# safijari/yag-slam

Measured on AMD Instinct MI355X. Metric: pose hypotheses/sec, higher is better.
Workload: dtype u8

## Files before the change

include/yagmatch.h:

```cpp
#ifndef YAGMATCH_H
#define YAGMATCH_H

#include <stdint.h>

#ifdef __cplusplus
extern "C" {
#endif

#define YM_VERSION 1

enum {
    YM_OK = 0,
    YM_ERR_INVALID = -1,
    YM_ERR_NO_DEVICE = -2,
    YM_ERR_HIP = -3,
    YM_ERR_UNSUPPORTED = -4,
    YM_ERR_RANGE = -5,
    YM_ERR_BUSY = -6
};

enum { YM_SEM_KARTO = 0, YM_SEM_YAGPY = 1 };

typedef struct ym_config {
    double angle_variance_penalty;
// ... 269 lines not shown
void ym_graph_destroy(ym_graph *g);
int ym_graph_add_nodes(ym_graph *g, const double *xyt, int n);
int ym_graph_add_constraints(ym_graph *g, const int32_t *from_to, const double *mean_xyt, const double *info9, int n);
int ym_graph_size(const ym_graph *g, int32_t *nodes, int32_t *constraints);
int ym_graph_set_poses(ym_graph *g, int first, const double *xyt, int n);
int ym_graph_get_poses(const ym_graph *g, int first, double *xyt, int n);
int ym_graph_hold(ym_graph *g, const int32_t *nodes, int n, int hold );
int ym_graph_held(const ym_graph *g, uint8_t *mask, int n_nodes);
int ym_graph_chi2(ym_graph *g, double *chi2);
int ym_graph_linearise(ym_graph *g, double *chi2, double *diag9 , double *grad3 );
int ym_graph_solve(ym_graph *g, int band , double lambda, double cg_tol, int max_cg_iters ,
                   double *delta3 , double *precond3 , int32_t *band_used,
                   int32_t *cg_iterations, double *residual, int32_t *flags);
typedef struct ym_opt_params { int32_t iters, exact, max_cg_iters, band ; double lambda0, cg_tol; } ym_opt_params;
typedef struct ym_opt_report { double chi2_initial, chi2_final, lambda_final; int32_t lm_steps, accepted, cg_iterations, band, status; } ym_opt_report;
int ym_graph_optimize(ym_graph *g, const ym_opt_params *p, ym_opt_report *out);

enum { YM_ROBUST_NONE = 0, YM_ROBUST_HUBER = 1, YM_ROBUST_CAUCHY = 2, YM_ROBUST_GEMAN_MCCLURE = 3 };
int ym_graph_set_robust(ym_graph *g, const int32_t *edges, int n, int kind, double param);
int ym_graph_enable(ym_graph *g, const int32_t *edges, int n, int enable );
int ym_graph_edge_terms(ym_graph *g, double *s , double *w );
int ym_graph_cost(ym_graph *g, double *cost);

typedef struct ym_grid_info {
    int32_t width, height, pitch;
    int32_t origin_x, origin_y;
    int32_t storage_w, storage_h;
    int32_t roi_x, roi_y, roi_w, roi_h;
    double offset_x, offset_y;
} ym_grid_info;
int ym_debug_grid_info(ym_matcher *m, int item, ym_grid_info *info);
int ym_debug_grid(ym_matcher *m, int item, uint8_t *out, int64_t out_bytes);
int ym_debug_sums(ym_matcher *m, int item, int pass, uint32_t *out, int64_t out_count);
int ym_debug_map_sums(ym_matcher *m, int item, int pass, uint32_t *out, int64_t out_count);
int ym_debug_query_local(ym_matcher *m, int item, double *out_xy, int32_t cap, int32_t *n);
int ym_debug_cells(ym_matcher *m, int item, int32_t *out, int64_t out_count, int32_t *max_n);
typedef struct ym_pair_list_info {
    int32_t nt, lnw, lparts, nbins;
    int32_t nrx, nry, nregions;
    int32_t rg_h, rg_cls, rg_zero;
    int32_t ng;
    int32_t qrep, cx0, cy0, nq;
    int32_t n_slots;
    int64_t entries_pstride;
    double off_x, off_y;
    double ylat[2];
} ym_pair_list_info;
int ym_debug_pair_lists(ym_matcher *m, int slot, ym_pair_list_info *info, double *ctrig, int32_t *starts, int32_t *flags,
                        uint16_t *entries, uint32_t *rbox);

int ym_debug_option(ym_matcher *m, int option, int value);

#define YM_DEBUG_COUNTERS 10
int ym_debug_counters(ym_matcher *m, int64_t *out, int32_t count);

int ym_debug_live_bytes(int64_t *device_bytes, int64_t *pinned_bytes);

int ym_debug_stamps(ym_matcher *m, int enable, uint64_t *out, int32_t count);

int ym_profile_enable(ym_matcher *m, int on);
int ym_profile_read(ym_matcher *m, int which, double *ms_total, int64_t *launches, int reset);
int ym_cache_stats(const ym_matcher *m, int64_t *hits, int64_t *misses);

#ifdef __cplusplus
}
#endif
// ... 2 lines not shown
```

yag_slam_amd/_capi.py:

```python
import ctypes as C
import os
import subprocess

_HERE = os.path.dirname(os.path.abspath(__file__))
LIB_PATH = os.environ.get("YM_LIB_PATH") or os.path.join(_HERE, "libyagmatch.so")

YM_OK = 0
SEM = {"karto": 0, "yagpy": 1}

EXPORTS = (
    "ym_version", "ym_build_id", "ym_device_count", "ym_last_error", "ym_create", "ym_destroy", "ym_get_config",
    "ym_set_stream", "ym_synchronize", "ym_scan_create", "ym_scans_create", "ym_scans_destroy", "ym_scan_set_pose", "ym_scans_set_poses", "ym_scan_get_pose",
    "ym_scan_size", "ym_scan_structure_trusted", "ym_scan_destroy", "ym_match", "ym_match_scans", "ym_map_sequence", "ym_process_scan", "ym_sequence_stats", "ym_async_slots",
    "ym_match_scans_async", "ym_wait", "ym_match_batch", "ym_batch_create", "ym_batch_destroy", "ym_batch_size",
    "ym_match_pairs", "ym_pairs_create",
    "ym_batch_run_async", "ym_batch_wait", "ym_debug_grid_info",
    "ym_debug_grid", "ym_debug_sums", "ym_debug_query_local", "ym_debug_cells", "ym_debug_pair_lists", "ym_debug_option", "ym_debug_stamps", "ym_debug_live_bytes",
    "ym_profile_enable",
    "ym_profile_read", "ym_cache_stats", "ym_debug_counters",
    "ym_coarse_dims", "ym_match_slice_begin", "ym_match_slice_finish",
    "ym_occupancy_create", "ym_occupancy_create_counted", "ym_occupancy_get_info", "ym_occupancy_read", "ym_occupancy_read_counts",
    "ym_occupancy_destroy", "ym_image_despeckle", "ym_occupancy_create_clean", "ym_occupancy_get_despeckle_stats",
    "ym_occmap_create", "ym_occmap_accumulate", "ym_occmap_clear", "ym_occmap_get_info", "ym_occmap_read", "ym_occmap_read_counts",
    "ym_occmap_debug_option", "ym_occmap_destroy",
    "ym_map_from_occupancy", "ym_map_from_grid", "ym_map_size", "ym_map_read", "ym_map_destroy", "ym_match_map",
    "ym_match_map_many", "ym_map_track", "ym_debug_map_sums", "ym_match_sets", "ym_match_sets_many",
    "ym_map_create_empty", "ym_map_add_scans", "ym_map_clear",
    "ym_map_create_counted", "ym_map_update_scans", "ym_map_counted", "ym_map_read_stamps",
    "ym_map_reframe", "ym_map_window", "ym_map_create_counted_window",
    "ym_raymap_create", "ym_raymap_trace", "ym_raymap_trace_each", "ym_raymap_destroy",
    "ym_locator_create", "ym_locator_get_info", "ym_locator_read_level", "ym_locator_locate", "ym_locator_destroy",
    "ym_segments_create", "ym_segments_label_range", "ym_segments_stats", "ym_segments_boundaries", "ym_segments_pairs",
    "ym_segments_destroy", "ym_map_free_space", "ym_segments_from_map", "ym_segments_labels",
    "ym_graph_create", "ym_graph_destroy", "ym_graph_add_nodes", "ym_graph_add_constraints", "ym_graph_size", "ym_graph_set_poses",
    "ym_graph_get_poses", "ym_graph_chi2", "ym_graph_linearise", "ym_graph_solve", "ym_graph_optimize",
    "ym_graph_hold", "ym_graph_held", "ym_graph_set_robust", "ym_graph_enable", "ym_graph_edge_terms", "ym_graph_cost",
)


class YmError(RuntimeError):
    def __init__(self, code, msg):
        super().__init__("libyagmatch error %d: %s" % (code, msg))
        self.code = code


class YmConfig(C.Structure):
    _fields_ = [
        ("angle_variance_penalty", C.c_double),
        ("distance_variance_penalty", C.c_double),
        ("coarse_search_angle_offset", C.c_double),
# ... 176 lines not shown
    L.ym_synchronize.argtypes = [vp]
    L.ym_scan_create.restype = vp
    L.ym_scan_create.argtypes = [C.c_int, C.POINTER(YmScanDesc)]
    L.ym_scan_set_pose.argtypes = [vp, C.c_double, C.c_double, C.c_double]
    L.ym_scans_set_poses.argtypes = [C.POINTER(vp), dp, C.c_int]
    L.ym_scan_get_pose.argtypes = [vp, dp]
    L.ym_scan_size.argtypes = [vp]
    L.ym_scan_destroy.argtypes = [vp]
    L.ym_scans_create.argtypes = [C.c_int, vp, C.c_int, vp]
    L.ym_scans_destroy.argtypes = [vp, C.c_int]
    L.ym_scans_destroy.restype = None
    L.ym_scan_destroy.restype = None
    L.ym_match.argtypes = [vp, C.POINTER(YmScanDesc), C.POINTER(YmScanDesc), C.c_int, C.c_int, C.c_int,
                           C.POINTER(YmResult)]
    L.ym_match_scans.argtypes = [vp, vp, C.POINTER(vp), C.c_int, C.c_int, C.c_int, C.POINTER(YmResult)]
    L.ym_async_slots.argtypes = [vp]
    L.ym_match_scans_async.argtypes = [vp, vp, C.POINTER(vp), C.c_int, C.c_int, C.c_int, C.c_int]
    L.ym_wait.argtypes = [vp, C.c_int, C.POINTER(YmResult)]
    L.ym_match_batch.argtypes = [vp, vp, C.POINTER(vp), ip, C.c_int, C.c_int, C.c_int, C.POINTER(YmResult),
                                 C.POINTER(YmResult), ip]
    L.ym_batch_create.restype = vp
    L.ym_batch_create.argtypes = [vp, vp, C.POINTER(vp), ip, C.c_int]
    L.ym_pairs_create.restype = vp
    L.ym_pairs_create.argtypes = [vp, C.POINTER(vp), C.POINTER(vp), ip, C.c_int]
    L.ym_match_pairs.argtypes = [vp, C.POINTER(vp), C.POINTER(vp), ip, C.c_int, C.c_int, C.c_int, C.POINTER(YmResult)]
    L.ym_batch_destroy.argtypes = [vp]
    L.ym_batch_destroy.restype = None
    L.ym_batch_size.argtypes = [vp]
    L.ym_batch_run_async.argtypes = [vp, vp, C.c_int, C.c_int, C.c_int, C.c_int64, vp]
    L.ym_batch_wait.argtypes = [vp, C.c_int, C.POINTER(YmResult), C.POINTER(YmResult), ip]
    L.ym_debug_grid_info.argtypes = [vp, C.c_int, C.POINTER(YmGridInfo)]
    L.ym_debug_grid.argtypes = [vp, C.c_int, C.POINTER(C.c_uint8), C.c_int64]
    L.ym_debug_sums.argtypes = [vp, C.c_int, C.c_int, C.POINTER(C.c_uint32), C.c_int64]
    L.ym_debug_query_local.argtypes = [vp, C.c_int, dp, C.c_int32, ip]
    L.ym_debug_cells.argtypes = [vp, C.c_int, ip, C.c_int64, ip]
    L.ym_debug_pair_lists.argtypes = [vp, C.c_int, C.POINTER(YmPairListInfo), dp, ip, ip, C.POINTER(C.c_uint16), C.POINTER(C.c_uint32)]
    L.ym_debug_option.argtypes = [vp, C.c_int, C.c_int]
    L.ym_debug_stamps.argtypes = [vp, C.c_int, C.POINTER(C.c_uint64), C.c_int32]
    L.ym_debug_live_bytes.argtypes = [C.POINTER(C.c_int64), C.POINTER(C.c_int64)]
    L.ym_profile_enable.argtypes = [vp, C.c_int]
    L.ym_profile_read.argtypes = [vp, C.c_int, dp, C.POINTER(C.c_int64), C.c_int]
    L.ym_cache_stats.argtypes = [vp, C.POINTER(C.c_int64), C.POINTER(C.c_int64)]
    L.ym_debug_counters.argtypes = [vp, C.POINTER(C.c_int64), C.c_int32]
    L.ym_coarse_dims.argtypes = [vp, ip]
    L.ym_scan_structure_trusted.argtypes = [vp, C.c_int]
    L.ym_process_scan.argtypes = [vp, vp, C.POINTER(vp), C.c_int, dp, dp, C.c_int, C.c_int, C.POINTER(YmResult)]
    L.ym_sequence_stats.argtypes = [vp, C.POINTER(C.c_int64), C.POINTER(C.c_int64), C.POINTER(C.c_int64)]
    L.ym_map_sequence.argtypes = [vp, C.POINTER(vp), dp, C.c_int, C.c_int, C.c_int, C.c_int, C.c_int, C.c_int, C.POINTER(YmResult), ip]
    L.ym_match_slice_begin.argtypes = [vp, vp, C.POINTER(vp), C.c_int, C.c_int, C.c_int, C.c_int, C.c_int, vp, vp]
    L.ym_match_slice_finish.argtypes = [vp, C.POINTER(YmResult)]
    L.ym_occupancy_create.restype = vp
    L.ym_occupancy_create.argtypes = [C.POINTER(vp), C.c_int, C.c_double, C.c_double]
    L.ym_occupancy_create_counted.restype = vp
    L.ym_occupancy_create_counted.argtypes = [C.POINTER(vp), C.c_int, C.c_double, C.c_double]
    L.ym_occupancy_get_info.argtypes = [vp, C.POINTER(YmOccupancyInfo)]
    L.ym_occupancy_read.argtypes = [vp, C.POINTER(C.c_uint8), C.c_int64]
    L.ym_occupancy_read_counts.argtypes = [vp, C.POINTER(C.c_uint32), C.POINTER(C.c_uint32), C.c_int64]
    L.ym_occupancy_destroy.argtypes = [vp]
    L.ym_occupancy_destroy.restype = None
    L.ym_image_despeckle.argtypes = [C.c_int, C.POINTER(C.c_uint8), C.c_int, C.c_int, C.c_int, C.POINTER(YmDespeckleOpts),
                                     C.POINTER(C.c_uint8), C.POINTER(YmDespeckleStats)]
    L.ym_occupancy_create_clean.restype = vp
    L.ym_occupancy_create_clean.argtypes = [C.POINTER(vp), C.c_int, C.c_double, C.c_double, C.POINTER(YmDespeckleOpts)]
    L.ym_occupancy_get_despeckle_stats.argtypes = [vp, C.POINTER(YmDespeckleStats)]
    L.ym_occmap_create.restype = vp
    L.ym_occmap_create.argtypes = [C.c_int, C.c_double, C.c_double, dp, C.c_int]
# ... 117 lines not shown
```

yag_slam_amd/csrc/ym_abi_debug.hpp:

```cpp
int ym_debug_map_sums(ym_matcher *m, int item, int pass, uint32_t *out, int64_t out_count);
static bool sets_debug(const ym_matcher *m) { return !m->last_valid && m->map_last.valid && m->sets_last.valid; }
int ym_debug_grid_info(ym_matcher *m, int item, ym_grid_info *info) {
    if (!m || !info) return set_err(YM_ERR_INVALID, "null argument");
    if (sets_debug(m)) {
        const ym_matcher::SetsLast &sl = m->sets_last;
        if (item < 0 || item >= m->map_last.n_items) return set_err(YM_ERR_INVALID, "no such item in the last call");
        std::memset(info, 0, sizeof *info);
        info->width = info->height = info->pitch = sl.G;
        info->storage_w = info->storage_h = info->roi_w = info->roi_h = sl.G;
        YmItemState s;
        DEV_GUARD(m->device);
        HIP_TRY(hipStreamSynchronize(m->stream));
        HIP_TRY(hipMemcpy(&s, m->states.p + item, sizeof s, hipMemcpyDeviceToHost));
        info->offset_x = s.off_x; info->offset_y = s.off_y;
        return YM_OK;
    }
    if (!m->last_valid || item < 0 || item >= m->last_B) return set_err(YM_ERR_INVALID, "no such item in the last call");
    const YmGeom &g = m->last_geom;
    info->width = g.win_w; info->height = g.win_w; info->pitch = g.pitch;
    info->origin_x = g.win_origin; info->origin_y = g.win_origin;
    info->storage_w = g.storage_w; info->storage_h = g.storage_w;
    info->roi_x = g.border; info->roi_y = g.border; info->roi_w = g.roi_w; info->roi_h = g.roi_w;
    YmItemState s;
    DEV_GUARD(m->device);
// ... 8 lines not shown
    if (sets_debug(m)) {
        const ym_matcher::SetsLast &sl = m->sets_last;
        if (item < 0 || item >= m->map_last.n_items) return set_err(YM_ERR_INVALID, "no such item in the last call");
        if (item < sl.first_grid) return set_err(YM_ERR_INVALID, "the grid of item %d was overwritten: the call keeps those of its last chunk, from item %d on", item, sl.first_grid);
        const int64_t need_s = (int64_t)sl.G * sl.G;
        if (out_bytes < need_s) return set_err(YM_ERR_INVALID, "grid buffer too small: need %lld bytes", (long long)need_s);
        DEV_GUARD(m->device);
        HIP_TRY(hipStreamSynchronize(m->stream));
        HIP_TRY(hipMemcpy(out, m->sets_grid.p + (size_t)(item - sl.first_grid) * sl.grid_stride, (size_t)need_s, hipMemcpyDeviceToHost));
        return YM_OK;
    }
    if (!m->last_valid || item < 0 || item >= m->last_B) return set_err(YM_ERR_INVALID, "no such item in the last call");
    const int64_t need = (int64_t)m->last_geom.pitch * m->last_geom.win_w;
    if (out_bytes < need) return set_err(YM_ERR_INVALID, "grid buffer too small: need %lld bytes", (long long)need);
    DEV_GUARD(m->device);
    HIP_TRY(hipStreamSynchronize(m->stream));
    HIP_TRY(hipMemcpy(out, m->grid.p + (size_t)item * m->last_grid_stride, (size_t)need, hipMemcpyDeviceToHost));
    return YM_OK;
}

int ym_debug_sums(ym_matcher *m, int item, int pass, uint32_t *out, int64_t out_count) {
    if (!m || !out || pass < 0 || pass > 1) return set_err(YM_ERR_INVALID, "bad argument");
    if (sets_debug(m)) return ym_debug_map_sums(m, item, pass, out, out_count);
    if (!m->last_valid || item < 0 || item >= m->last_B) return set_err(YM_ERR_INVALID, "no such item in the last call");
    const size_t n = m->last_sums_stride[pass];
    if (n == 0) return set_err(YM_ERR_INVALID, "pass %d did not run", pass);
    const size_t ncopy = std::min(n, (size_t)out_count);
    if (m->cfg.semantics == YM_SEM_KARTO && (size_t)out_count < n)
        return set_err(YM_ERR_INVALID, "sums buffer too small: need %zu entries", n);
    DEV_GUARD(m->device);
    HIP_TRY(hipStreamSynchronize(m->stream));
    HIP_TRY(hipMemcpy(out, m->sums.p + m->sums_pass_offset[pass] + (size_t)item * n, ncopy * sizeof(uint32_t),
                      hipMemcpyDeviceToHost));
    return YM_OK;
}

int ym_debug_query_local(ym_matcher *m, int item, double *out_xy, int32_t cap, int32_t *n) {
    if (!m || !out_xy || !n) return set_err(YM_ERR_INVALID, "null argument");
    const bool sets = sets_debug(m);
    if (sets ? (item < 0 || item >= m->map_last.n_items) : (!m->last_valid || item < 0 || item >= m->last_B))
        return set_err(YM_ERR_INVALID, "no such item in the last call");
    YmItemState s;
    DEV_GUARD(m->device);
    HIP_TRY(hipStreamSynchronize(m->stream));
    HIP_TRY(hipMemcpy(&s, m->states.p + item, sizeof s, hipMemcpyDeviceToHost));
    *n = s.nq;
    if (cap < s.nq) return set_err(YM_ERR_INVALID, "buffer too small: need %d points", s.nq);
    if (s.nq > 0)
        HIP_TRY(hipMemcpy(out_xy, s.ql, sizeof(double2) * s.nq, hipMemcpyDeviceToHost));
    return YM_OK;
}

int ym_debug_cells(ym_matcher *m, int item, int32_t *out, int64_t out_count, int32_t *max_n) {
    if (!m || !max_n) return set_err(YM_ERR_INVALID, "null argument");
    if (!m->last_valid || item < 0 || item >= m->last_B) return set_err(YM_ERR_INVALID, "no such item in the last call");
    *max_n = m->last_max_n;
    const size_t per = (size_t)m->last_max_base * m->last_max_n;
    if (!out) return YM_OK;
    if ((size_t)out_count < per * 2) return set_err(YM_ERR_INVALID, "buffer too small: need %zu ints", per * 2);
    DEV_GUARD(m->device);
    HIP_TRY(hipStreamSynchronize(m->stream));
    std::vector<YmCell> dev(per);
    HIP_TRY(hipMemcpy(dev.data(), m->cells.p + (size_t)item * per, sizeof(YmCell) * per, hipMemcpyDeviceToHost));
    for (size_t i = 0; i < per; i++) {
        const int2 c = ym_cell_unpack(dev[i]);
        out[2 * i] = c.x;
// ... 201 lines not shown
```

yag_slam_amd/csrc/ym_host_call.hpp:

```cpp
int launch_call_body(ym_matcher *m, Slot &slot) {
    static const bool debug_host = getenv("YM_DEBUG_HOST") != nullptr;
    timespec t_[8];
    auto mark = [&](int i) { if (debug_host) clock_gettime(CLOCK_MONOTONIC, &t_[i]); };
    mark(7);
    DEV_GUARD(m->device);
    CallPlan P;
    int rc;
    mark(0);
    m->last_corr_form = -1;
    m->lists_last.valid = false;
    if ((rc = plan_sizes(m, slot, P))) return rc;
    mark(1);
    Call &pc = slot.call;
    const bool replay = pc.batch_uid != 0 && pc.plan_clean && pc.plan_gen == m->cache_gen && pc.pose_epoch == g_pose_epoch.load(std::memory_order_relaxed);
    if (!replay && (rc = plan_cache(m, slot, P))) return rc;
    mark(2);
    if ((rc = plan_jobs(m, slot, P, replay))) return rc;
    mark(3);
    if ((rc = plan_descriptor(m, slot, P, replay))) return rc;
    if (pc.batch_uid != 0 && !replay) {
        bool clean = !m->cache_off;
        for (const CallScan &cs : pc.scans) clean = clean && !cs.stale && !cs.qstale;
        pc.plan_clean = clean;
        pc.plan_gen = m->cache_gen;
// ... 42 lines not shown
        emark(4);
        if (!slot.call.slice) enqueue_finish(m, slot, P);
        else slot.plan = P;
        emark(5);
    }
    if (slot.dev_best_out)
        hipLaunchKernelGGL(ym::argbest_kernel, dim3(1), dim3(256), 0, st, m->states.p, P.B, (long long)slot.chain_id_base,
                           reinterpret_cast<double *>(slot.dev_best_out));
    HIP_TRY(hipGetLastError());
    if ((rc = prof_end(m, ev_call))) return rc;
    if (!slot.done) HIP_TRY(hipEventCreateWithFlags(&slot.done, hipEventDisableTiming));
    if (!slot.call.chain_step) HIP_TRY(hipEventRecord(slot.done, st));
    slot.in_flight = true;
    slot.n_items = P.B;
    HIP_TRY(hipGetLastError());
    mark(6);
    if (debug_host) {
        auto us = [&](int a, int b) { return (t_[b].tv_sec - t_[a].tv_sec) * 1e6 + (t_[b].tv_nsec - t_[a].tv_nsec) * 1e-3; };
        fprintf(stderr, "[ym] host us: guard %.1f sizes %.0f cache %.0f jobs %.0f descriptor %.0f raster-plan %.0f enqueue %.0f (B %d, %d scans)\n", us(7, 0), us(0, 1), us(1, 2),
                us(2, 3), us(3, 4), us(4, 5), us(5, 6), P.B, P.nscans);
        auto eus = [&](int a, int b) { return (e_[b].tv_sec - e_[a].tv_sec) * 1e6 + (e_[b].tv_nsec - e_[a].tv_nsec) * 1e-3; };
        fprintf(stderr, "[ym] enqueue us: prepare %.1f raster %.1f correlate %.1f score %.1f finish %.1f\n", eus(0, 1), eus(1, 2), eus(2, 3), eus(3, 4), eus(4, 5));
    }

    m->last_geom = P.g;
    m->last_lat[0] = P.lc;
    m->last_lat[1] = P.lf;
    m->last_B = P.B; m->last_max_n = P.max_n; m->last_max_base = P.max_base;
    m->last_nt_stride = P.nt_stride; m->last_dim_stride = P.dim_stride;
    m->last_grid_stride = P.grid_stride;
    m->last_sums_stride[0] = P.yag ? P.yvol : (m->keep_sums || (P.B < 8 && P.sums_c <= 65536)) ? P.sums_c : 0;
    m->last_sums_stride[1] = slot.call.refine ? (P.yag ? P.yvol : P.sums_f) : 0;
    m->last_valid = true;
    if (P.region26 && P.k_end > P.k_begin) {
        const ym::RegionArgs r = region_args(m, P);
        ym_matcher::ListsLast &ll = m->lists_last;
        ll.nt = P.lc.nt; ll.lnw = r.nw; ll.lparts = r.parts; ll.nbins = r.nbins; ll.nrx = r.nrx; ll.nry = r.nry; ll.nregions = r.nregions;
        ll.rg_h = r.rg_h; ll.rg_cls = r.rg_cls; ll.rg_zero = r.rg_zero; ll.ng = r.ng;
        ll.entries_pstride = r.entries_pstride; ll.entries_stride = r.entries_stride; ll.starts_stride = r.starts_stride; ll.rbox_stride = r.rbox_stride;
        ll.qrep.swap(P.qrep);
        ll.valid = true;
    }
    return YM_OK;
}

int launch_call(ym_matcher *m, Slot &slot) {
    const uint64_t before = m->call_counter;
    const int rc = launch_call_body(m, slot);
    if (rc != YM_OK) {
        if (m->side_stream && m->ev_join && hipEventRecord(m->ev_join, m->side_stream) == hipSuccess)
            (void)hipStreamWaitEvent(m->stream, m->ev_join, 0);
        if (m->call_counter != before)
            for (ym_matcher::CacheEntry &ce : m->cache_entries)
                if (ce.stale_in_call == m->call_counter) ce.pose[0] = ce.pose[1] = ce.pose[2] = std::nan("");
        slot.desc_live_bytes = 0;
        slot.call.plan_clean = false;
        slot.in_flight = false;
        m->list_key_valid = false;
    }
    return rc;
}

void state_to_result(const ym_matcher *m, const Slot &slot, const YmItemState &s, int expansions, int64_t prior_hyp,
                     ym_result *r) {
    std::memset(r, 0, sizeof *r);
    r->response = s.response;
// ... 226 lines not shown
```

yag_slam_amd/csrc/ym_host_matcher.hpp:

```cpp
struct ym_map {
    int device;
    int width, height;
    DevBuf<double> d_cgrid;
    DevBuf<uint8_t> d_g8;
    int x0 = 0, y0 = 0;
    bool counted = false;
    double ox = 0, oy = 0;
    DevBuf<uint32_t> d_stamps;
    DevBuf<uint8_t> d_dirty;
};

struct ym_occupancy {
    int device;
    ym_occupancy_info info;
    std::vector<uint8_t> image;
    std::vector<uint32_t> counts;
    bool cleaned = false;
    ym_despeckle_stats clean_stats{};
};

struct ym_occmap {
    int device = 0;
    double resolution = 0, range_threshold = 0, scale = 0;
    bool has_anchor = false, added = false;
// ... 136 lines not shown
    DevBuf<uint4> sel_rec;
    DevBuf<unsigned> sel_slot;
    DevBuf<uint32_t> tile_list;
    DevBuf<int32_t> tile_count;
    DevBuf<int32_t> tile_max;
    DevBuf<uint16_t> tile_hits;
    PinnedBuf tile_max_host;
    int finish_form = 0;
    int corr_chunks = 0;
    int corr_pad_lds = 0;
    int corr_cw = 0;
    int corr_dedup = 0;
    int corr_region = 0;
    int corr_region_na = 0;
    int corr_region_parts = 0;
    int corr_region_cap = 0;
    int corr_region_lds = 0;
    int raster_gx = 0;
    int raster_hits_per_tile = 0;
    int keep_sums = 0;
    int finish_threads = 0;
    int force_regather = 0;
    int select_global = 0;
    int select_split_max = 8;
    DevBuf<double> tmp_ranges;
    PinnedBuf tmp_ranges_host;
    Slot slots[kAsyncSlots + 1];
    YmGeom last_geom;
    YmLattice last_lat[2];
    int last_B = 0, last_max_n = 0, last_max_base = 0, last_nt_stride = 0, last_dim_stride = 0;
    size_t last_grid_stride = 0, last_sums_stride[2] = {0, 0};
    size_t sums_pass_offset[2] = {0, 0};
    bool last_valid = false;
    struct ListsLast {
        bool valid = false;
        int32_t nt = 0, lnw = 0, lparts = 0, nbins = 0, nrx = 0, nry = 0, nregions = 0, rg_h = 0, rg_cls = 0, rg_zero = 0, ng = 0;
        size_t entries_pstride = 0, entries_stride = 0, starts_stride = 0, rbox_stride = 0;
        std::vector<int32_t> qrep;
    } lists_last;
    bool profiling = false;
    ProfEvents prof[3];
};
```

yag_slam_amd/csrc/ym_k_common.hpp:

```cpp
#pragma once

namespace ym {

__device__ __forceinline__ double kt_round(double v) { return v >= 0.0 ? floor(v + 0.5) : ceil(v - 0.5); }
__device__ __forceinline__ bool kt_double_equal(double a, double b) {
    double d = a - b;
    return d < 0.0 ? d >= -YM_KT_TOLERANCE : d <= YM_KT_TOLERANCE;
}
__device__ inline double kt_normalize_angle(double angle) {
    while (angle < -YM_KT_PI) {
        if (angle < -YM_KT_2PI) angle += (double)(unsigned int)(angle / -YM_KT_2PI) * YM_KT_2PI;
        else angle += YM_KT_2PI;
    }
    while (angle > YM_KT_PI) {
        if (angle > YM_KT_2PI) angle -= (double)(unsigned int)(angle / YM_KT_2PI) * YM_KT_2PI;
        else angle -= YM_KT_2PI;
    }
    return angle;
}
__device__ inline double kt_normalize_angle_difference(double minuend, double subtrahend) {
    while (minuend - subtrahend < -YM_KT_PI) minuend += YM_KT_2PI;
    while (minuend - subtrahend > YM_KT_PI) minuend -= YM_KT_2PI;
    return minuend;
}
__device__ __forceinline__ int kt_round_int(double v) {
    const int r = (int)(fabs(v) + 0.5);
    return v < 0.0 ? -r : r;
}
__device__ __forceinline__ int world_to_grid(double w, double off, double scale) {
    return kt_round_int((w - off) * scale);
}

__device__ __forceinline__ int block_scan_flag(bool flag, int *total, int *wave_counts) {
    const int lane = threadIdx.x & 63, w = threadIdx.x >> 6, nw = (blockDim.x + 63) >> 6;
    unsigned long long m = __ballot(flag);
    int pre = __popcll(m & ((1ull << lane) - 1ull));
    if (lane == 0) wave_counts[w] = __popcll(m);
    __syncthreads();
    int base = 0, tot = 0;
    for (int i = 0; i < nw; i++) {
        int c = wave_counts[i];
// ... 144 lines not shown
```

yag_slam_amd/csrc/ym_k_finish.hpp:

```cpp
#pragma once

namespace ym {

#define YM_SCORE_THREADS 256
struct ScoreArgs {
    YmGeom g;
    YmLattice lat;
    const uint16_t *partial;
    size_t partial_stride;
    const YmItemState *states;
    uint32_t *sums;
    size_t sums_stride;
    double *resp;
    double *blockmax;
    double *probs;
    size_t probs_stride;
    int32_t n_chunks, nx_pad, n_blocks;
    int32_t k_begin, k_end;
    int32_t write_blockmax;
    int32_t lane_layout;
    unsigned long long *stamps;
};

__device__ __forceinline__ double dist_penalty(const YmGeom &g, double sq_dist) {
    double dp = 1.0 - (YM_PENALTY_GAIN * sq_dist / g.dist_var);
    return dp > g.min_dist_pen ? dp : g.min_dist_pen;
}
__device__ __forceinline__ double hyp_response_dp(const YmGeom &g, int penalize, unsigned sum, int nq, double dp,
                                                  double angle, double center_t) {
    double response = 0.0;
    if (nq != 0) {
        response = (double)sum;
        response /= (double)(nq * YM_OCCUPIED);
    }
    if (penalize && !kt_double_equal(response, 0.0)) {
        const double sq_ang = (angle - center_t) * (angle - center_t);
        double ap = 1.0 - (YM_PENALTY_GAIN * sq_ang / g.ang_var);
        ap = ap > g.min_ang_pen ? ap : g.min_ang_pen;
        response *= (dp * ap);
    }
    return response;
}
__device__ __forceinline__ double hyp_response(const YmGeom &g, int penalize, unsigned sum, int nq, double sq_dist,
                                               double angle, double center_t) {
    return hyp_response_dp(g, penalize, sum, nq, dist_penalty(g, sq_dist), angle, center_t);
}

__device__ __forceinline__ int2 lattice_cell(const YmLattice &L, int c) {
    const int iy = c / L.nx;
    return make_int2(c - iy * L.nx, iy);
}
__device__ __forceinline__ double2 lattice_xy(const YmLattice &L, int2 ic) {
    return make_double2(-L.off_x + ic.x * L.step_x, -L.off_y + ic.y * L.step_y);
}
__device__ __forceinline__ int2 lattice_hyp(const YmLattice &L, int h) {
    const int nxy = L.nx * L.ny, k = h / nxy;
    return make_int2(k, h - k * nxy);
}

__device__ __forceinline__ const uint16_t *cell_partials(const ScoreArgs &a, int b, int k, int2 ic, size_t *kstride, size_t *cstride) {
    *kstride = a.lane_layout ? (size_t)64 * 16 : (size_t)a.lat.ny * a.nx_pad;
    *cstride = (size_t)a.lat.nt * *kstride;
    return a.partial + (size_t)b * a.partial_stride + (size_t)k * *kstride +
           (a.lane_layout ? (size_t)((32 * (ic.x / 13) + ic.y) * 16 + ic.x % 13) : (size_t)ic.y * a.nx_pad + ic.x);
}
template <int UNROLL>
__device__ __forceinline__ unsigned chunk_group_sum(const uint16_t *p, int n_chunks, size_t cstride) {
    unsigned sum = 0;
#pragma unroll UNROLL
    for (int c2 = 0; c2 < n_chunks; c2++) sum += p[(size_t)c2 * cstride];
    return sum;
}

__global__ __launch_bounds__(YM_SCORE_THREADS) void score_kernel(ScoreArgs a) {
// ... 685 lines not shown
```

yag_slam_amd/csrc/ym_k_region.hpp:

```cpp
#pragma once

namespace ym {

#ifndef YM_RG_PROF
#define YM_RG_PROF 0
#endif
#if YM_RG_PROF
#if YM_RG_PROF == 2
#define YM_RG_PH(i) do { if ((i) == 7 || (i) == 8 || (i) == 1 || (i) == 2 || (i) == 5) { const uint32_t t_ = (uint32_t)__builtin_amdgcn_s_memtime(); \
    if ((i) != 5) ph[(i) == 7 ? 0 : (i) == 8 ? 1 : (i) == 1 ? 2 : 3] += t_ - pt; pt = t_; } } while (0)
#else
#define YM_RG_PH(i) do { const uint32_t t_ = (uint32_t)__builtin_amdgcn_s_memtime(); if ((i) >= 2 && (i) <= 5) ph[(i) - 2] += t_ - pt; pt = t_; } while (0)
#endif
#else
#define YM_RG_PH(i) do { } while (0)
#endif

#ifndef YM_RG_ABLATE
#define YM_RG_ABLATE 0
#endif
#ifndef YM_RG_PRIO
#define YM_RG_PRIO 0
#endif
#define YM_RG_W 64
// ... 556 lines not shown
    YM_STAMP(a, 9);
#endif
#if YM_RG_PROF
    auto prof_out = [&]() {
        if (a.stamps && lane == 0) {
            for (int i = 0; i < 4; i++) atomicAdd(a.stamps + 10 + i, (unsigned long long)ph[i]);
            atomicAdd(a.stamps + 8, (unsigned long long)(pt - pt_begin));
            atomicAdd(a.stamps + 9, __builtin_amdgcn_s_memrealtime() - rt_begin);
        }
    };
#endif
    if (!a.fuse_score) {
        if (!kvalid) return;
        while (flushed < ng) flush();
        return;
    }
    unsigned long long *pmax = reinterpret_cast<unsigned long long *>(region);
    const int nxy = nx * ny;
    double *dpen = reinterpret_cast<double *>(region) + ((nxy + 1) & ~1);
    __syncthreads();
    for (int i = tid; i < nxy; i += NT) {
        pmax[i] = 0ull;
        const int iy = i / nx, ix = i - iy * nx;
        const double x = -a.lat.off_x + ix * a.lat.step_x, y = -a.lat.off_y + iy * a.lat.step_y;
        dpen[i] = dist_penalty(a.g, x * x + y * y);
    }
    __syncthreads();
    if (kvalid) {
        unsigned tot[YM_RG_G];
        rg_odd(acc);
#pragma unroll
        for (int j = 0; j < YM_RG_G; j++) tot[j] = (acc[2 * (j >> 2) + (j & 1)] >> (16 * ((j >> 1) & 1))) & 0xffffu;
        for (int f = 0; f < min(flushed, ng); f++) {
            const uint16_t *pp = a.partial + (size_t)b * a.partial_stride + (((size_t)f * nt + k) * 64 + lane) * 16;
#pragma unroll
            for (int j = 0; j < YM_RG_G; j++) tot[j] += pp[j];
        }
        const double ct = st.center[2];
        const int nq = st.nq;
        const double angle = (ct - a.lat.angle_off) + k * a.lat.angle_res;
        const int ncb = (nxy + YM_SCORE_THREADS - 1) / YM_SCORE_THREADS;
        double bmax0 = -1.0, bmax1 = -1.0;
        const int c0 = row * nx + half * YM_RG_G, cb0 = job ? c0 / YM_SCORE_THREADS : 0;
#pragma unroll
        for (int j = 0; j < YM_RG_G; j++) {
            const int ix = half * YM_RG_G + j;
            if (job && ix < nx) {
                const int c = row * nx + ix;
                const double r = hyp_response_dp(a.g, a.lat.penalize, tot[j], nq, dpen[c], angle, ct);
                a.resp[(size_t)b * a.sums_stride + (size_t)k * nxy + c] = r;
                if (c / YM_SCORE_THREADS == cb0) bmax0 = r > bmax0 ? r : bmax0;
                else bmax1 = r > bmax1 ? r : bmax1;
                if (r > 0.0) atomicMax(&pmax[c], (unsigned long long)__double_as_longlong(r));
            }
        }
        for (int cb = 0; cb < ncb; cb++) {
            const double mine = !job ? -1.0 : cb == cb0 ? bmax0 : cb == cb0 + 1 ? bmax1 : -1.0;
            const double m = wave_reduce(mine, OpMaxD());
            if (lane == 0) a.blockmax[(size_t)b * a.n_blocks + (size_t)k * ncb + cb] = m;
        }
    }
    __syncthreads();
    for (int i = tid; i < nxy; i += NT)
        if (pmax[i]) atomicMax(reinterpret_cast<unsigned long long *>(a.probs) + (size_t)b * a.probs_stride + i, pmax[i]);
#if YM_RG_PROF
    YM_RG_PH(6);
    prof_out();
#endif
}

}
```

yag_slam_amd/scan_matching.py:

```python
import ctypes as C
import os
import struct
from collections import namedtuple

import numpy as np

from . import _capi
from .config import default_config, default_config_loop, make_config
from .models import LocalizedRangeScan
from .transform import Transform

ScanMatcherResult = namedtuple('ScanMatcherResult', ['response', 'covariance', 'best_pose', 'meta'])


def _pose_of(scan):
    p = scan.corrected_pose
    return float(p.x), float(p.y), float(p.euler[-1])


def _desc_of(scan, keep):
    d = _capi.YmScanDesc()
    r = np.ascontiguousarray(scan.ranges, dtype=np.float64)
    keep.append(r)
    d.ranges = r.ctypes.data_as(C.POINTER(C.c_double))
# ... 507 lines not shown
        poses = _move_rigidly([m_.corrected_pose for m_ in moved], c0[0], c0[1], c1[0], c1[1], c1[2] - c0[2])
        return ScanMatcherResult(r.response, r.covariance, poses, meta)

    def match_scan_async(self, query, base_scans, penalty=True, do_fine=False, slot=0):
        hq = self._require_native(query)
        arr = (C.c_void_p * max(1, len(base_scans)))(*self._handles(base_scans))
        _capi.check(self._lib.ym_match_scans_async(self._m, hq, arr, len(base_scans), int(bool(penalty)),
                                                   int(bool(do_fine)), int(slot)))

    def wait(self, slot=0):
        res = _capi.YmResult()
        _capi.check(self._lib.ym_wait(self._m, int(slot), C.byref(res)))
        return _result(res)

    def synchronize(self):
        _capi.check(self._lib.ym_synchronize(self._m))

    def set_stream(self, stream_handle):
        _capi.check(self._lib.ym_set_stream(self._m, C.c_void_p(stream_handle) if stream_handle else None))

    def debug_grid(self, item=0):
        info = _capi.YmGridInfo()
        _capi.check(self._lib.ym_debug_grid_info(self._m, item, C.byref(info)))
        buf = np.zeros((info.height, info.pitch), dtype=np.uint8)
        _capi.check(self._lib.ym_debug_grid(self._m, item, buf.ctypes.data_as(C.POINTER(C.c_uint8)), buf.size))
        return buf[:, :info.width], info

    def debug_sums(self, pass_=0, item=0, dims=None):
        nx, ny, nt = dims
        buf = np.zeros((nt, ny, nx), dtype=np.uint32)
        _capi.check(self._lib.ym_debug_sums(self._m, item, pass_, buf.ctypes.data_as(C.POINTER(C.c_uint32)), buf.size))
        return buf

    def debug_map_sums(self, pass_=0, item=0, dims=None):
        nx, ny, nt = dims
        buf = np.zeros((nt, ny, nx), dtype=np.uint32)
        _capi.check(self._lib.ym_debug_map_sums(self._m, int(item), int(pass_), buf.ctypes.data_as(C.POINTER(C.c_uint32)), buf.size))
        return buf

    def debug_query_local(self, item=0, cap=8192):
        buf = np.zeros((cap, 2))
        n = C.c_int32()
        _capi.check(self._lib.ym_debug_query_local(self._m, item, buf.ctypes.data_as(C.POINTER(C.c_double)), cap,
                                                   C.byref(n)))
        return buf[:n.value].copy()

    def debug_cells(self, item=0, cap=1 << 16):
        buf = np.zeros((cap, 2), dtype=np.int32)
        max_n = C.c_int32()
        _capi.check(self._lib.ym_debug_cells(self._m, item, buf.ctypes.data_as(C.POINTER(C.c_int32)), buf.size,
                                             C.byref(max_n)))
        return buf.reshape(-1, 2), max_n.value

    def debug_pair_lists(self, slot=0):
        info = _capi.YmPairListInfo()
        none = (None,) * 5
        _capi.check(self._lib.ym_debug_pair_lists(self._m, int(slot), C.byref(info), *none))
        ctrig = np.zeros((info.nt, 2))
        starts = np.zeros((info.lparts, info.nbins + 1), dtype=np.int32)
        flags = np.zeros(info.lparts, dtype=np.int32)
        entries = np.zeros((info.lparts, info.entries_pstride), dtype=np.uint16)
        rbox = np.zeros((info.nregions, info.lparts), dtype=np.uint32)
        _capi.check(self._lib.ym_debug_pair_lists(self._m, int(slot), C.byref(info), ctrig.ctypes.data_as(C.POINTER(C.c_double)),
                                                  starts.ctypes.data_as(C.POINTER(C.c_int32)), flags.ctypes.data_as(C.POINTER(C.c_int32)),
                                                  entries.ctypes.data_as(C.POINTER(C.c_uint16)), rbox.ctypes.data_as(C.POINTER(C.c_uint32))))
        out = {n: int(getattr(info, n)) for n, _ in _capi.YmPairListInfo._fields_[:17]}
# ... 431 lines not shown
```

Before: 14.70 billion.

## Replace per-hypothesis division with reciprocal-multiply scoring and vectorized partial loads

The region kernel's scoring epilogue now computes each response as the sum times a precomputed reciprocal with an FMA correction, instead of a double division per hypothesis. The zero check becomes an integer test, and the angle penalty is hoisted out of the per-cell loop. Partial-sum reads become two 128-bit loads, and a wave-uniform fast path skips bounds and range checks when all lanes are full and in range. A debug entry point is added to read back responses, block maxima and probabilities so the new arithmetic can be checked for exactness against the old division.

```diff
diff --git a/include/yagmatch.h b/include/yagmatch.h
--- a/include/yagmatch.h
+++ b/include/yagmatch.h
@@ -325,6 +325,8 @@
 int ym_debug_grid_info(ym_matcher *m, int item, ym_grid_info *info);
 int ym_debug_grid(ym_matcher *m, int item, uint8_t *out, int64_t out_bytes);
 int ym_debug_sums(ym_matcher *m, int item, int pass, uint32_t *out, int64_t out_count);
+int ym_debug_scores(ym_matcher *m, int item, double *resp, int64_t resp_count, double *blockmax, int64_t blockmax_count, double *probs,
+                    int64_t probs_count);
 int ym_debug_map_sums(ym_matcher *m, int item, int pass, uint32_t *out, int64_t out_count);
 int ym_debug_query_local(ym_matcher *m, int item, double *out_xy, int32_t cap, int32_t *n);
 int ym_debug_cells(ym_matcher *m, int item, int32_t *out, int64_t out_count, int32_t *max_n);
diff --git a/yag_slam_amd/_capi.py b/yag_slam_amd/_capi.py
--- a/yag_slam_amd/_capi.py
+++ b/yag_slam_amd/_capi.py
@@ -15,7 +15,7 @@
     "ym_match_scans_async", "ym_wait", "ym_match_batch", "ym_batch_create", "ym_batch_destroy", "ym_batch_size",
     "ym_match_pairs", "ym_pairs_create",
     "ym_batch_run_async", "ym_batch_wait", "ym_debug_grid_info",
-    "ym_debug_grid", "ym_debug_sums", "ym_debug_query_local", "ym_debug_cells", "ym_debug_pair_lists", "ym_debug_option", "ym_debug_stamps", "ym_debug_live_bytes",
+    "ym_debug_grid", "ym_debug_sums", "ym_debug_scores", "ym_debug_query_local", "ym_debug_cells", "ym_debug_pair_lists", "ym_debug_option", "ym_debug_stamps", "ym_debug_live_bytes",
     "ym_profile_enable",
     "ym_profile_read", "ym_cache_stats", "ym_debug_counters",
     "ym_coarse_dims", "ym_match_slice_begin", "ym_match_slice_finish",
@@ -258,6 +258,7 @@
     L.ym_debug_grid_info.argtypes = [vp, C.c_int, C.POINTER(YmGridInfo)]
     L.ym_debug_grid.argtypes = [vp, C.c_int, C.POINTER(C.c_uint8), C.c_int64]
     L.ym_debug_sums.argtypes = [vp, C.c_int, C.c_int, C.POINTER(C.c_uint32), C.c_int64]
+    L.ym_debug_scores.argtypes = [vp, C.c_int, C.POINTER(C.c_double), C.c_int64, C.POINTER(C.c_double), C.c_int64, C.POINTER(C.c_double), C.c_int64]
     L.ym_debug_query_local.argtypes = [vp, C.c_int, dp, C.c_int32, ip]
     L.ym_debug_cells.argtypes = [vp, C.c_int, ip, C.c_int64, ip]
     L.ym_debug_pair_lists.argtypes = [vp, C.c_int, C.POINTER(YmPairListInfo), dp, ip, ip, C.POINTER(C.c_uint16), C.POINTER(C.c_uint32)]
diff --git a/yag_slam_amd/csrc/ym_abi_debug.hpp b/yag_slam_amd/csrc/ym_abi_debug.hpp
--- a/yag_slam_amd/csrc/ym_abi_debug.hpp
+++ b/yag_slam_amd/csrc/ym_abi_debug.hpp
@@ -64,6 +64,24 @@
     HIP_TRY(hipStreamSynchronize(m->stream));
     HIP_TRY(hipMemcpy(out, m->sums.p + m->sums_pass_offset[pass] + (size_t)item * n, ncopy * sizeof(uint32_t),
                       hipMemcpyDeviceToHost));
+    return YM_OK;
+}
+
+int ym_debug_scores(ym_matcher *m, int item, double *resp, int64_t resp_count, double *blockmax, int64_t blockmax_count, double *probs,
+                    int64_t probs_count) {
+    if (!m) return set_err(YM_ERR_INVALID, "null argument");
+    if (!m->last_valid || item < 0 || item >= m->last_B) return set_err(YM_ERR_INVALID, "no such item in the last call");
+    if (!m->last_resp || !m->last_probs) return set_err(YM_ERR_INVALID, "the last call kept no Karto responses");
+    const YmLattice &lc = m->last_lat[0];
+    const size_t nxy = (size_t)lc.nx * lc.ny, vol = nxy * lc.nt, nb = (size_t)m->last_score_blocks;
+    if (vol > m->last_resp_stride) return set_err(YM_ERR_INVALID, "the last call's lattice does not fit its response volume");
+    if ((resp && (size_t)resp_count < vol) || (blockmax && (size_t)blockmax_count < nb) || (probs && (size_t)probs_count < nxy))
+        return set_err(YM_ERR_INVALID, "scores buffer too small: need %zu responses, %zu block maxima, %zu cells", vol, nb, nxy);
+    DEV_GUARD(m->device);
+    HIP_TRY(hipStreamSynchronize(m->stream));
+    if (resp) HIP_TRY(hipMemcpy(resp, m->last_resp + (size_t)item * m->last_resp_stride, vol * sizeof(double), hipMemcpyDeviceToHost));
+    if (blockmax) HIP_TRY(hipMemcpy(blockmax, m->blockmax.p + (size_t)item * nb, nb * sizeof(double), hipMemcpyDeviceToHost));
+    if (probs) HIP_TRY(hipMemcpy(probs, m->last_probs + (size_t)item * nxy, nxy * sizeof(double), hipMemcpyDeviceToHost));
     return YM_OK;
 }
 
diff --git a/yag_slam_amd/csrc/ym_host_call.hpp b/yag_slam_amd/csrc/ym_host_call.hpp
--- a/yag_slam_amd/csrc/ym_host_call.hpp
+++ b/yag_slam_amd/csrc/ym_host_call.hpp
@@ -98,6 +98,7 @@
     m->last_sums_stride[0] = P.yag ? P.yvol : (m->keep_sums || (P.B < 8 && P.sums_c <= 65536)) ? P.sums_c : 0;
     m->last_sums_stride[1] = slot.call.refine ? (P.yag ? P.yvol : P.sums_f) : 0;
     m->last_valid = true;
+    m->last_resp = P.yag ? nullptr : P.resp; m->last_probs = P.probs; m->last_resp_stride = P.sums_c; m->last_score_blocks = P.score_blocks;
     if (P.region26 && P.k_end > P.k_begin) {
         const ym::RegionArgs r = region_args(m, P);
         ym_matcher::ListsLast &ll = m->lists_last;
diff --git a/yag_slam_amd/csrc/ym_host_matcher.hpp b/yag_slam_amd/csrc/ym_host_matcher.hpp
--- a/yag_slam_amd/csrc/ym_host_matcher.hpp
+++ b/yag_slam_amd/csrc/ym_host_matcher.hpp
@@ -192,6 +192,9 @@
     size_t last_grid_stride = 0, last_sums_stride[2] = {0, 0};
     size_t sums_pass_offset[2] = {0, 0};
     bool last_valid = false;
+    const double *last_resp = nullptr, *last_probs = nullptr;
+    size_t last_resp_stride = 0;
+    int last_score_blocks = 0;
     struct ListsLast {
         bool valid = false;
         int32_t nt = 0, lnw = 0, lparts = 0, nbins = 0, nrx = 0, nry = 0, nregions = 0, rg_h = 0, rg_cls = 0, rg_zero = 0, ng = 0;
diff --git a/yag_slam_amd/csrc/ym_k_common.hpp b/yag_slam_amd/csrc/ym_k_common.hpp
--- a/yag_slam_amd/csrc/ym_k_common.hpp
+++ b/yag_slam_amd/csrc/ym_k_common.hpp
@@ -1,12 +1,9 @@
 #pragma once
+#include "ym_score_rule.hpp"
 
 namespace ym {
 
 __device__ __forceinline__ double kt_round(double v) { return v >= 0.0 ? floor(v + 0.5) : ceil(v - 0.5); }
-__device__ __forceinline__ bool kt_double_equal(double a, double b) {
-    double d = a - b;
-    return d < 0.0 ? d >= -YM_KT_TOLERANCE : d <= YM_KT_TOLERANCE;
-}
 __device__ inline double kt_normalize_angle(double angle) {
     while (angle < -YM_KT_PI) {
         if (angle < -YM_KT_2PI) angle += (double)(unsigned int)(angle / -YM_KT_2PI) * YM_KT_2PI;
diff --git a/yag_slam_amd/csrc/ym_k_finish.hpp b/yag_slam_amd/csrc/ym_k_finish.hpp
--- a/yag_slam_amd/csrc/ym_k_finish.hpp
+++ b/yag_slam_amd/csrc/ym_k_finish.hpp
@@ -26,20 +26,20 @@
     double dp = 1.0 - (YM_PENALTY_GAIN * sq_dist / g.dist_var);
     return dp > g.min_dist_pen ? dp : g.min_dist_pen;
 }
+__device__ __forceinline__ double angle_penalty(const YmGeom &g, double angle, double center_t) {
+    const double sq_ang = (angle - center_t) * (angle - center_t);
+    const double ap = 1.0 - (YM_PENALTY_GAIN * sq_ang / g.ang_var);
+    return ap > g.min_ang_pen ? ap : g.min_ang_pen;
+}
+template <bool CHECKED>
+__device__ __forceinline__ double hyp_response_pen(int penalize, unsigned sum, const ScoreDivisor &sd, double dp, double ap) {
+    double response = CHECKED ? score_quotient_checked(sum, sd) : score_quotient(sum, sd);
+    if (penalize && !(CHECKED ? sum == 0u : score_is_zero(sum, response, sd))) response *= (dp * ap);
+    return response;
+}
 __device__ __forceinline__ double hyp_response_dp(const YmGeom &g, int penalize, unsigned sum, int nq, double dp,
                                                   double angle, double center_t) {
-    double response = 0.0;
-    if (nq != 0) {
-        response = (double)sum;
-        response /= (double)(nq * YM_OCCUPIED);
-    }
-    if (penalize && !kt_double_equal(response, 0.0)) {
-        const double sq_ang = (angle - center_t) * (angle - center_t);
-        double ap = 1.0 - (YM_PENALTY_GAIN * sq_ang / g.ang_var);
-        ap = ap > g.min_ang_pen ? ap : g.min_ang_pen;
-        response *= (dp * ap);
-    }
-    return response;
+    return hyp_response_pen<false>(penalize, sum, score_divisor(nq), dp, angle_penalty(g, angle, center_t));
 }
 __device__ __forceinline__ double hyp_response(const YmGeom &g, int penalize, unsigned sum, int nq, double sq_dist,
                                                double angle, double center_t) {
diff --git a/yag_slam_amd/csrc/ym_k_region.hpp b/yag_slam_amd/csrc/ym_k_region.hpp
--- a/yag_slam_amd/csrc/ym_k_region.hpp
+++ b/yag_slam_amd/csrc/ym_k_region.hpp
@@ -612,28 +612,53 @@
 #pragma unroll
         for (int j = 0; j < YM_RG_G; j++) tot[j] = (acc[2 * (j >> 2) + (j & 1)] >> (16 * ((j >> 1) & 1))) & 0xffffu;
         for (int f = 0; f < min(flushed, ng); f++) {
-            const uint16_t *pp = a.partial + (size_t)b * a.partial_stride + (((size_t)f * nt + k) * 64 + lane) * 16;
-#pragma unroll
-            for (int j = 0; j < YM_RG_G; j++) tot[j] += pp[j];
+            const uint4 *pp = reinterpret_cast<const uint4 *>(a.partial + (size_t)b * a.partial_stride + (((size_t)f * nt + k) * 64 + lane) * 16);
+            const uint4 lo = pp[0], hi = pp[1];
+            const uint32_t w[8] = {lo.x, lo.y, lo.z, lo.w, hi.x, hi.y, hi.z, hi.w};
+#pragma unroll
+            for (int j = 0; j < YM_RG_G; j++) tot[j] += (w[j >> 1] >> (16 * (j & 1))) & 0xffffu;
         }
         const double ct = st.center[2];
-        const int nq = st.nq;
+        const ScoreDivisor sd = score_divisor(st.nq);
         const double angle = (ct - a.lat.angle_off) + k * a.lat.angle_res;
+        const double apen = angle_penalty(a.g, angle, ct);
+        const int penalize = a.lat.penalize;
         const int ncb = (nxy + YM_SCORE_THREADS - 1) / YM_SCORE_THREADS;
         double bmax0 = -1.0, bmax1 = -1.0;
         const int c0 = row * nx + half * YM_RG_G, cb0 = job ? c0 / YM_SCORE_THREADS : 0;
-#pragma unroll
-        for (int j = 0; j < YM_RG_G; j++) {
-            const int ix = half * YM_RG_G + j;
-            if (job && ix < nx) {
-                const int c = row * nx + ix;
-                const double r = hyp_response_dp(a.g, a.lat.penalize, tot[j], nq, dpen[c], angle, ct);
-                a.resp[(size_t)b * a.sums_stride + (size_t)k * nxy + c] = r;
-                if (c / YM_SCORE_THREADS == cb0) bmax0 = r > bmax0 ? r : bmax0;
-                else bmax1 = r > bmax1 ? r : bmax1;
-                if (r > 0.0) atomicMax(&pmax[c], (unsigned long long)__double_as_longlong(r));
-            }
-        }
+        const int nv = job ? min(YM_RG_G, nx - half * YM_RG_G) : 0;
+        const int js = (cb0 + 1) * YM_SCORE_THREADS - c0;
+        double *rp = a.resp + (size_t)b * a.sums_stride + (size_t)k * nxy + c0;
+        const double *dp = dpen + c0;
+        unsigned long long *pm = pmax + c0;
+        unsigned top_sum = tot[0];
+#pragma unroll
+        for (int j = 1; j < YM_RG_G; j++) top_sum = max(top_sum, tot[j]);
+        auto score_lane = [&](auto full) {
+            constexpr bool FULL = decltype(full)::value;
+            if (nv != 0) {
+                double dpj[YM_RG_G];
+#pragma unroll
+                for (int j = 0; j < YM_RG_G; j++) dpj[j] = FULL || j < nv ? dp[j] : 1.0;
+#pragma unroll
+                for (int j = 0; j < YM_RG_G; j++) {
+                    if (FULL || j < nv) {
+#if YM_RG_ABLATE & 8
+                        const double r = 0.0;
+#else
+                        const double r = hyp_response_pen<FULL>(penalize, tot[j], sd, dpj[j], apen);
+#endif
+                        rp[j] = r;
+                        const bool lo = j < js;
+                        bmax0 = (lo && r > bmax0) ? r : bmax0;
+                        bmax1 = (!lo && r > bmax1) ? r : bmax1;
+                        if (r > 0.0) atomicMax(&pm[j], (unsigned long long)__double_as_longlong(r));
+                    }
+                }
+            }
+        };
+        if (__any(nv != 0 && (nv != YM_RG_G || top_sum > sd.top))) score_lane(std::false_type());
+        else score_lane(std::true_type());
         for (int cb = 0; cb < ncb; cb++) {
             const double mine = !job ? -1.0 : cb == cb0 ? bmax0 : cb == cb0 + 1 ? bmax1 : -1.0;
             const double m = wave_reduce(mine, OpMaxD());
diff --git a/yag_slam_amd/csrc/ym_score_rule.hpp b/yag_slam_amd/csrc/ym_score_rule.hpp
--- /dev/null
+++ b/yag_slam_amd/csrc/ym_score_rule.hpp
@@ -0,0 +1,53 @@
+#pragma once
+#include <math.h>
+
+#if defined(__HIPCC__) || defined(__CUDACC__)
+#define YM_SCORE_FN __host__ __device__ __forceinline__
+#else
+#define YM_SCORE_FN inline
+#endif
+
+namespace ym {
+
+constexpr int kScoreOccupied = 100;
+constexpr int kScoreMaxBeams = 6000;
+constexpr double kScoreTolerance = 1e-06;
+#if defined(YM_OCCUPIED) && defined(YM_MAX_BEAMS) && defined(YM_KT_TOLERANCE)
+static_assert(kScoreOccupied == YM_OCCUPIED && kScoreMaxBeams == YM_MAX_BEAMS && kScoreTolerance == YM_KT_TOLERANCE,
+              "ym_score_rule.hpp restates ym_types.h");
+#endif
+
+YM_SCORE_FN bool kt_double_equal(double a, double b) {
+    double d = a - b;
+    return d < 0.0 ? d >= -kScoreTolerance : d <= kScoreTolerance;
+}
+
+struct ScoreDivisor {
+    double d;
+    double y;
+    unsigned top;
+    int nq;
+};
+YM_SCORE_FN ScoreDivisor score_divisor(int nq) {
+    ScoreDivisor s;
+    s.nq = nq;
+    s.d = (double)(nq * kScoreOccupied);
+    s.y = nq != 0 ? 1.0 / s.d : 0.0;
+    s.top = nq > 0 && nq <= kScoreMaxBeams ? (unsigned)(nq * kScoreOccupied) : 0u;
+    return s;
+}
+YM_SCORE_FN double score_quotient_checked(unsigned sum, const ScoreDivisor &s) {
+    const double a = (double)sum;
+    const double q0 = a * s.y;
+    const double r = fma(-q0, s.d, a);
+    return fma(r, s.y, q0);
+}
+YM_SCORE_FN double score_quotient(unsigned sum, const ScoreDivisor &s) {
+    if (sum <= s.top) return score_quotient_checked(sum, s);
+    return s.nq != 0 ? (double)sum / s.d : 0.0;
+}
+YM_SCORE_FN bool score_is_zero(unsigned sum, double response, const ScoreDivisor &s) {
+    return s.top ? sum == 0u : kt_double_equal(response, 0.0);
+}
+
+}
diff --git a/yag_slam_amd/scan_matching.py b/yag_slam_amd/scan_matching.py
--- a/yag_slam_amd/scan_matching.py
+++ b/yag_slam_amd/scan_matching.py
@@ -563,6 +563,15 @@
         _capi.check(self._lib.ym_debug_sums(self._m, item, pass_, buf.ctypes.data_as(C.POINTER(C.c_uint32)), buf.size))
         return buf
 
+    def debug_scores(self, item=0, dims=None):
+        nx, ny, nt = dims
+        resp, probs = np.zeros((nt, ny, nx)), np.zeros((ny, nx))
+        blockmax = np.zeros((nt, (nx * ny + 255) // 256))
+        dp = C.POINTER(C.c_double)
+        _capi.check(self._lib.ym_debug_scores(self._m, int(item), resp.ctypes.data_as(dp), resp.size, blockmax.ctypes.data_as(dp),
+                                              blockmax.size, probs.ctypes.data_as(dp), probs.size))
+        return resp, blockmax, probs
+
     def debug_map_sums(self, pass_=0, item=0, dims=None):
         nx, ny, nt = dims
         buf = np.zeros((nt, ny, nx), dtype=np.uint32)
```

Result: no change. 14.76 billion, median of 6 (+0.4%).
